# Intsights/PySubstringSearch

Measured on AMD Instinct MI355X. Metric: queries/sec (batched) + index-build GB/s on 512MB chunk, 1/2/4/8 GPU, higher is better.
Workload: dtype u64

## Files before the change

### pysubstringsearch_amd/csrc/msd_sort.hip

```cpp
#include "msd_sort.h"

#include <algorithm>
#include <type_traits>
#include <vector>

#include "prims.h"
#include "scan.h"
#include "text_keys.h"

namespace pss {

constexpr int MSD_D = 10;
constexpr u32 MSD_BINS = 1u << MSD_D;
constexpr int MSD_BLOCK = 512;
constexpr int MSD_WAVES = MSD_BLOCK / kWave;
constexpr int MSD_IPT = 16;
constexpr u32 MSD_TILE = MSD_BLOCK * MSD_IPT;
constexpr u32 MSD_WIN = 6144;
#ifndef PSS_LS_WINDOW
#define PSS_LS_WINDOW 8
#endif
constexpr u32 MSD_TILE_CAP = 8184 - PSS_LS_WINDOW;
constexpr u32 MSD_MAX_BUCKET = 4088;
constexpr int MSD_TAG_BITS = MSD_D + 1;
// ... 382 lines not shown
#pragma unroll
        for (int k = 0; k < MSD_IPT; ++k) {
            const u32 p = k * MSD_BLOCK + tid;
            if (p < valid) {
                u64 e = exch[p];
                u32 d;
                if (FROM_TEXT) {
                    d = (u32)(e >> 13) & (MSD_BINS - 1u);
                    e = ((e >> 23) << a.idx_bits) | (u64)(base + ((u32)e & (MSD_TILE - 1u)));
                } else {
                    d = (u32)(e >> shift2) & (MSD_BINS - 1u);
                    e = (e & low_mask2) | ((u64)(hist[d] >> 16) << shift2);
                }
                a.out[s_delta[d] + p] = e;
            }
        }
    }
}

constexpr u32 MSD_TILE2 = 16384;
constexpr int MSD_PIECES2 = MSD_TILE2 / MSD_TILE;

template <bool FROM_TEXT, int BLOCK, bool LSD = false>
__global__ __launch_bounds__(BLOCK) void msd_scatter2_kernel(MsdArgs a)
{
    constexpr int IPT = MSD_TILE2 / BLOCK;
    constexpr int BPT = MSD_BINS / BLOCK;
    __shared__ __attribute__((aligned(16))) u64 exch[MSD_TILE];
    __shared__ u32 hist[MSD_BINS], s_delta[MSD_BINS], s_off[MSD_BINS];
    __shared__ u16 s_start[MSD_BINS];
    __shared__ u32 scr[BLOCK / kWave + 1];
    const u32 tid = threadIdx.x, r = blockIdx.x;
    u32 e0, e1;
    u32 tag[BPT];
#pragma unroll
    for (int j = 0; j < BPT; ++j) tag[j] = 0;
    if (FROM_TEXT) {
        if (r >= a.num_ranges1) return;
        e0 = r * a.tiles_per_range1 * MSD_TILE;
        const u64 end = (u64)(r + 1) * a.tiles_per_range1 * MSD_TILE;
        e1 = end < a.n ? (u32)end : a.n;
    } else {
        if (r >= a.counters[0]) return;
        e0 = a.ranges2[r].start;
        e1 = a.ranges2[r].end;
#pragma unroll
        for (int j = 0; j < BPT; ++j)
            tag[j] = ((u32)a.dense[(size_t)a.ranges2[r].seg * MSD_BINS + BPT * tid + j] & (MSD_TAG_SPAN - 1u)) << 16;
    }
#pragma unroll
    for (int j = 0; j < BPT; ++j) {
        const u32 i = BPT * tid + j;
        hist[i] = tag[j];
        s_off[i] = FROM_TEXT ? a.T[(size_t)i * a.num_ranges1 + r] + a.J1[i] : a.T[(size_t)r * MSD_BINS + i];
    }
    __syncthreads();
    const int shift2 = a.idx_bits + a.key_bits - 2 * MSD_D;
    const u64 low_mask2 = (1ull << shift2) - 1ull;
    const int rest_bits = a.key_bits - MSD_D;
    const u64 rest_mask = (1ull << rest_bits) - 1ull;
    for (u32 base = e0; base < e1; base += MSD_TILE2) {
        const u32 valid = min(MSD_TILE2, e1 - base);
        u64 elem[IPT];
        u32 lp[IPT];
        if (FROM_TEXT) {
#pragma unroll
            for (int g = 0; g < IPT / 16; ++g) {
                const u32 i0 = base + tid * IPT + g * 16;
                u64 key[16] = {};
                if (i0 < a.n) text_keys16(a.codes, i0, a.code_bits, a.key_chars, a.plus_one, a.key_drop, a.n, key);
#pragma unroll
                for (int k = 0; k < 16; ++k) {
                    const u32 pos = tid * IPT + g * 16 + k;
                    u32 d;
                    u64 keep;
                    if (LSD) {
                        d = (u32)(key[k] >> (rest_bits - MSD_D)) & (MSD_BINS - 1u);
                        keep = ((key[k] >> rest_bits) << (rest_bits - MSD_D)) | (key[k] & (rest_mask >> MSD_D));
                    } else {
                        d = (u32)(key[k] >> rest_bits) & (MSD_BINS - 1u);
                        keep = key[k] & rest_mask;
                    }
                    elem[g * 16 + k] = (keep << 24) | ((u64)d << 14) | (u64)pos;
                    lp[g * 16 + k] = pos < valid ? ((atomicAdd(&hist[d], 1u) & 0xffffu) | (d << 22)) : 0xffffffffu;
                }
            }
        } else {
#pragma unroll
            for (int k = 0; k < IPT; ++k) {
                const u32 p = k * BLOCK + tid;
                elem[k] = p < valid ? a.in[base + p] : 0ull;
            }
#pragma unroll
            for (int k = 0; k < IPT; ++k) {
                const u32 p = k * BLOCK + tid;
                const u32 d = (u32)(elem[k] >> shift2) & (MSD_BINS - 1u);
                lp[k] = p < valid ? ((atomicAdd(&hist[d], 1u) & 0xffffu) | (d << 22)) : 0xffffffffu;
            }
        }
        __syncthreads();
        {
            u32 c[BPT], sum = 0;
#pragma unroll
            for (int j = 0; j < BPT; ++j) {
                c[j] = hist[BPT * tid + j] & 0xffffu;
                sum += c[j];
            }
            u32 ex = block_excl_sum<BLOCK / kWave>(sum, scr, nullptr);
#pragma unroll
            for (int j = 0; j < BPT; ++j) {
                const u32 i = BPT * tid + j;
                s_start[i] = (u16)ex;
                const u32 o = s_off[i];
                s_delta[i] = o - ex;
                s_off[i] = o + c[j];
                hist[i] = tag[j];
                ex += c[j];
            }
        }
        __syncthreads();
#pragma unroll
        for (int k = 0; k < IPT; ++k)
            if (lp[k] != 0xffffffffu) lp[k] = (lp[k] & 0xffffu) + (u32)s_start[lp[k] >> 22];
#pragma unroll
        for (int h = 0; h < MSD_PIECES2; ++h) {
            if (h * MSD_TILE >= valid) break;
            if (h) __syncthreads();
#pragma unroll
            for (int k = 0; k < IPT; ++k) {
                const u32 q = lp[k] - h * MSD_TILE;
                if (q < MSD_TILE) exch[q] = elem[k];
            }
            __syncthreads();
#pragma unroll
            for (int k = 0; k < (int)(MSD_TILE / BLOCK); ++k) {
                const u32 q = k * BLOCK + tid, p = h * MSD_TILE + q;
                if (p < valid) {
                    u64 e = exch[q];
                    u32 d;
                    if (FROM_TEXT) {
                        d = (u32)(e >> 14) & (MSD_BINS - 1u);
                        e = ((e >> 24) << a.idx_bits) | (u64)(base + ((u32)e & (MSD_TILE2 - 1u)));
                    } else {
                        d = (u32)(e >> shift2) & (MSD_BINS - 1u);
                        e = (e & low_mask2) | ((u64)(hist[d] >> 16) << shift2);
                    }
                    a.out[s_delta[d] + p] = e;
                }
            }
        }
    }
}

constexpr u32 LB_A = 1u << 30, LB_P = 2u << 30, LB_STATE = 3u << 30, LB_VALUE = LB_A - 1u;
constexpr int LB_WINDOW = 4;

struct LbAsk {
    u32 v[LB_WINDOW];
};
__device__ __forceinline__ void lb_ask(const u32 *status, u32 p, LbAsk &q)
{
#pragma unroll
    for (u32 w = 0; w < (u32)LB_WINDOW; ++w) {
        const u32 r = p > w ? p - 1 - w : 0u;
        q.v[w] = __hip_atomic_load(&status[(size_t)r * MSD_BINS + threadIdx.x], __ATOMIC_RELAXED, __HIP_MEMORY_SCOPE_AGENT);
    }
}
__device__ __forceinline__ void lb_begin(u32 *status, u32 t, u32 c, LbAsk &q)
{
    if (t == 0) return;
    __hip_atomic_store(&status[(size_t)t * MSD_BINS + threadIdx.x], LB_A | c, __ATOMIC_RELAXED, __HIP_MEMORY_SCOPE_AGENT);
    lb_ask(status, t, q);
}
__device__ __forceinline__ u32 lb_finish(u32 *status, u32 t, u32 c, u32 first, LbAsk &q)
{
    u32 off = first;
    if (t != 0) {
        u32 sum = 0, p = t;
        for (;;) {
            const u32 p0 = p;
            bool stop = false, done = false;
#pragma unroll
            for (u32 w = 0; w < (u32)LB_WINDOW; ++w) {
                if (!stop && w < p0) {
                    const u32 st = q.v[w] & LB_STATE;
                    if (st == 0) {
                        stop = true;
                    } else {
                        sum += q.v[w] & LB_VALUE;
                        --p;
                        if (st == LB_P) done = stop = true;
                    }
                }
            }
            if (done || p == 0) break;
            lb_ask(status, p, q);
        }
        off = sum;
    }
    __hip_atomic_store(&status[(size_t)t * MSD_BINS + threadIdx.x], LB_P | (off + c), __ATOMIC_RELAXED, __HIP_MEMORY_SCOPE_AGENT);
    return off;
}


__global__ __launch_bounds__(MSD_BINS) void msd_tiles2_kernel(const u32 *J1, MsdTile2 *tiles, u32 *counters)
{
    __shared__ u32 scr[MSD_BINS / kWave + 1];
    const u32 d = threadIdx.x;
    const u32 s = J1[d], e = J1[d + 1];
    const u32 nr = (e - s + MSD_TILE2 - 1) / MSD_TILE2;
    u32 total = 0, D = 0;
    const u32 first = block_excl_sum<MSD_BINS / kWave>(nr, scr, &total);
    const u32 dn = block_excl_sum<MSD_BINS / kWave>(nr ? 1u : 0u, scr, &D);
    if (d == 0) counters[0] = total + (MSD_BINS - D);
    if (nr == 0) {
        const u32 dd = D + (d - dn);
        tiles[total + (d - dn)] = MsdTile2{s, 0u, dd | 0x80000000u};
    }
    for (u32 k = 0; k < nr; ++k) {
        const u32 ts = s + k * MSD_TILE2;
        tiles[first + k] = MsdTile2{ts, min(MSD_TILE2, e - ts), dn | (k + 1 == nr ? 0x80000000u : 0u)};
    }
}

__global__ __launch_bounds__(1024) void msd_scatter_lb_kernel(MsdArgs a)
{
    constexpr int BLOCK = 1024;
    constexpr int IPT = MSD_TILE2 / BLOCK;
    __shared__ __attribute__((aligned(16))) u64 exch[MSD_TILE];
    __shared__ u32 hist[MSD_BINS], s_delta[MSD_BINS];
    __shared__ u16 s_start[MSD_BINS];
    __shared__ u32 scr[BLOCK / kWave + 1];
    __shared__ u32 s_ticket;
    const u32 tid = threadIdx.x;
    const u32 nt = a.counters[0];
    const int shift2 = a.idx_bits + a.key_bits - 2 * MSD_D;
    const u64 low_mask2 = (1ull << shift2) - 1ull;
    hist[tid] = 0;
    __syncthreads();
    for (;;) {
        if (tid == 0) s_ticket = atomicAdd(&a.counters[8], 1u);
        __syncthreads();
        const u32 t = s_ticket;
        if (t >= nt) break;
        const MsdTile2 td = a.tiles2[t];
        const u32 base = td.start, valid = td.count;
        u64 elem[IPT];
        u32 lp[IPT];
#pragma unroll
        for (int k = 0; k < IPT; ++k) {
            const u32 p = k * BLOCK + tid;
            elem[k] = p < valid ? a.in[base + p] : 0ull;
        }
#pragma unroll
        for (int k = 0; k < IPT; ++k) {
            const u32 p = k * BLOCK + tid;
            const u32 d = (u32)(elem[k] >> shift2) & (MSD_BINS - 1u);
            lp[k] = p < valid ? (atomicAdd(&hist[d], 1u) | (d << 22)) : 0xffffffffu;
        }
        __syncthreads();
        const u32 c = hist[tid];
        LbAsk ask;
        lb_begin(a.status, t, c, ask);
        const u32 ex = block_excl_sum<BLOCK / kWave>(c, scr, nullptr);
        s_start[tid] = (u16)ex;
        hist[tid] = 0;
        __syncthreads();
        const u64 tag = (u64)(td.d_last & (MSD_RAW_TAG_SPAN - 1u)) << shift2;
#pragma unroll
        for (int k = 0; k < IPT; ++k)
            if (lp[k] != 0xffffffffu) lp[k] = (lp[k] & 0xffffu) + (u32)s_start[lp[k] >> 22];
#pragma unroll
        for (int h = 0; h < MSD_PIECES2; ++h) {
            if (h && h * MSD_TILE >= valid) break;
            if (h) __syncthreads();
#pragma unroll
            for (int k = 0; k < IPT; ++k) {
                const u32 q = lp[k] - h * MSD_TILE;
                if (q < MSD_TILE) exch[q] = elem[k];
            }
            if (h == 0) {
                if (t == 0 && tid == 0) a.J[0] = 0;
                const u32 off = lb_finish(a.status, t, c, a.Jb[tid], ask);
                if (td.d_last >> 31) a.J[(size_t)tid * MSD_BINS + (td.d_last & (MSD_BINS - 1u)) + 1u] = off + c;
                s_delta[tid] = off - ex;
            }
            __syncthreads();
#pragma unroll
            for (int k = 0; k < (int)(MSD_TILE / BLOCK); ++k) {
                const u32 q = k * BLOCK + tid, p = h * MSD_TILE + q;
                if (p < valid) {
                    const u64 e = exch[q];
                    const u32 d = (u32)(e >> shift2) & (MSD_BINS - 1u);
                    a.out[s_delta[d] + p] = (e & low_mask2) | tag;
                }
            }
        }
    }
}


struct InNonEmpty {
    const u32 *J;
    __device__ u64 operator()(u64 j) const { return J[j + 1] > J[j] ? 1u : 0u; }
};

// ... 665 lines not shown

#include "ss_sort_impl.h"


static size_t msd_max_tiles(uint32_t n)
{
    return (size_t)n / (SS_WIN / 2) + ((size_t)MSD_BINS * MSD_BINS) / MSD_RAW_TAG_SPAN + 8;
}

static size_t msd_max_tiles2(uint32_t n) { return (size_t)n / MSD_TILE2 + MSD_BINS + 8; }

static bool msd_use_lsd(uint32_t n)
{
    const char *e = knob("PSS_MSD_LSD");
    return !(e && atoi(e) == 0) && n < (1u << 30);
}

size_t msd_workspace_bytes(uint32_t n)
{
    const size_t max_ranges2 = (size_t)n / MSD_G2_RANGE + MSD_BINS + 8;
    const size_t nbk = (size_t)MSD_BINS * MSD_BINS;
    return max_ranges2 * MSD_BINS * 4
           + (MSD_BINS + 8) * 4
           + (nbk + 8) * 4
           + max_ranges2 * sizeof(MsdRange) + (MSD_BINS + 8) * 4 + 64
           + (nbk + 8) * 8
           + (nbk + 8) * 4
           + (msd_max_tiles(n) + 32) * 8
           + (msd_max_tiles(n) + 32) * 16
           + (msd_max_tiles(n) + 32) * sizeof(MsdTile)
           + (SC_MAX_BLOCKS + 8) * 8 + 8192
           + (size_t)MSD_BINS * MSD_G1_RANGES * 4 + (MSD_BINS + 8) * 4
           + msd_max_tiles2(n) * (sizeof(MsdTile2) + (size_t)MSD_BINS * 4)
           + (nbk + 8) * 4 + 4096;
}

int msd_max_key_bits(uint32_t n)
{
    int ib = 1;
    while ((1ull << ib) < (u64)n) ++ib;
    const int after2 = 64 + MSD_D - (msd_use_lsd(n) ? MSD_RAW_TAG_BITS : MSD_TAG_BITS) - ib + MSD_D;
    return std::min(after2, 64 + MSD_D - ib);
}

int msd_suffix_sort(DeviceCtx *ctx, const TextKeys *text, uint32_t n, int key_bits, uint64_t *A[2], uint32_t *sa_out,
                    void *work, uint32_t *h_small, bool profile, MsdStats *stats, bool *accepted, MsdActive *active,
                    const MsdFront *front)
{
    *accepted = false;
    hipStream_t s = ctx->stream;
    int ib = 1;
    while ((1ull << ib) < (u64)n) ++ib;
    if (key_bits < 2 * MSD_D + 1 || key_bits > msd_max_key_bits(n) || n < 2) {
        set_error("msd_suffix_sort: key of %d bits does not fit (n = %u)", key_bits, n);
        return PSS_EINVAL;
    }
    const size_t max_ranges2 = (size_t)n / MSD_G2_RANGE + MSD_BINS + 8;
    const size_t nbk = (size_t)MSD_BINS * MSD_BINS;
    u8 *w = static_cast<u8 *>(work);
    size_t o = 0;
    auto carve = [&](size_t bytes) { u8 *p = w + o; o = round_up(o + bytes, 256); return p; };
    u32 *T = reinterpret_cast<u32 *>(carve(max_ranges2 * MSD_BINS * 4));
    u32 *J1 = reinterpret_cast<u32 *>(carve((MSD_BINS + 8) * 4));
    u32 *J = reinterpret_cast<u32 *>(carve((nbk + 8) * 4));
    MsdRange *ranges2 = reinterpret_cast<MsdRange *>(carve(max_ranges2 * sizeof(MsdRange)));
    u32 *seg_first = reinterpret_cast<u32 *>(carve((MSD_BINS + 8) * 4));
    u32 *counters = reinterpret_cast<u32 *>(carve(64));
    u64 *ranks = reinterpret_cast<u64 *>(carve((nbk + 8) * 8));
    u32 *cstart = reinterpret_cast<u32 *>(carve((nbk + 8) * 4));
    const size_t max_tiles = msd_max_tiles(n);
    MsdTile *tiles_all = reinterpret_cast<MsdTile *>(carve((max_tiles + 16) * sizeof(MsdTile)));
    u32 *tile_first = reinterpret_cast<u32 *>(carve((max_tiles + 16) * 8));
    u32 *blk_cnt = reinterpret_cast<u32 *>(carve((max_tiles + 8) * 4));
    u64 *dst_off = reinterpret_cast<u64 *>(carve((max_tiles + 8) * 8));
    u64 *partial = reinterpret_cast<u64 *>(carve((SC_MAX_BLOCKS + 8) * 8));
    u64 *d_total = partial + SC_MAX_BLOCKS;
    const bool lsd = msd_use_lsd(n);
    const size_t max_tiles2 = msd_max_tiles2(n);
    u32 *T2 = nullptr, *Jb = nullptr, *status = nullptr, *cj = nullptr;
    MsdTile2 *tiles2 = nullptr;
    if (lsd) {
        T2 = reinterpret_cast<u32 *>(carve((size_t)MSD_BINS * MSD_G1_RANGES * 4));
        Jb = reinterpret_cast<u32 *>(carve((MSD_BINS + 8) * 4));
        tiles2 = reinterpret_cast<MsdTile2 *>(carve(max_tiles2 * sizeof(MsdTile2)));
        status = reinterpret_cast<u32 *>(carve(max_tiles2 * MSD_BINS * 4));
        cj = reinterpret_cast<u32 *>(carve((nbk + 8) * 4));
    }

    MsdArgs a;
    memset(&a, 0, sizeof a);
    a.codes = text->codes;
    a.code_bits = text->code_bits;
    a.key_chars = text->key_chars;
    a.plus_one = text->plus_one;
    a.key_drop = text->drop;
    a.n = n;
    a.key_bits = key_bits;
    a.idx_bits = ib;
    const u32 num_tiles = (u32)(((u64)n + MSD_TILE - 1) / MSD_TILE);
    a.tiles_per_range1 = (num_tiles + MSD_G1_RANGES - 1) / MSD_G1_RANGES;
    a.num_ranges1 = (num_tiles + a.tiles_per_range1 - 1) / a.tiles_per_range1;
    a.T = T;
    a.J1 = J1;
    a.J = J;
    a.ranges2 = ranges2;
    a.seg_first = seg_first;
    a.counters = counters;
    a.lsd = lsd ? 1 : 0;
    a.T2 = T2;
    a.Jb = Jb;
    a.tiles2 = tiles2;
    a.status = status;

    hipEvent_t ev[8] = {};
    int nev = 0;
    struct EvGuard {
        hipEvent_t *e;
        int *n;
        ~EvGuard()
        {
            for (int i = 0; i < *n; ++i) (void)hipEventDestroy(e[i]);
        }
    } guard{ev, &nev};
    auto mark = [&]() -> int {
        if (profile && nev < 8) {
            PSS_HIP(hipEventCreate(&ev[nev]));
            PSS_HIP(hipEventRecord(ev[nev], s));
            ++nev;
        }
        return PSS_OK;
    };

    PSS_HIP(hipMemsetAsync(counters, 0, 64, s));
    a.out = A[0];
    if (front) {
        a.raw = front->raw;
        a.lut = front->lut;
        a.codes_out = const_cast<u8 *>(text->codes);
        a.bad = front->bad;
        hipLaunchKernelGGL(msd_hist_raw_kernel, dim3(a.num_ranges1), dim3(MSD_BLOCK), 0, s, a);
    } else {
        hipLaunchKernelGGL(msd_hist_kernel<true>, dim3(a.num_ranges1), dim3(MSD_BLOCK), 0, s, a);
    }
    static_assert(MSD_G1_RANGES <= 1024, "msd_offsets1_kernel takes four ranges per thread");
    hipLaunchKernelGGL(msd_offsets1_kernel, dim3(MSD_BINS), dim3(256), 0, s, T, a.num_ranges1, seg_first);
    hipLaunchKernelGGL(msd_offsets1b_kernel, dim3(1), dim3(MSD_BINS), 0, s, (const u32 *)seg_first, J1, n);
    if (lsd) {
        hipLaunchKernelGGL(msd_offsets1_kernel, dim3(MSD_BINS), dim3(256), 0, s, T2, a.num_ranges1, seg_first);
        hipLaunchKernelGGL(msd_offsets1b_kernel, dim3(1), dim3(MSD_BINS), 0, s, (const u32 *)seg_first, Jb, n);
        PSS_HIP(hipMemsetAsync(status, 0, max_tiles2 * MSD_BINS * 4, s));
    }
    PSS_TRY(mark());
    const bool wide = lsd || !(knob("PSS_MSD_SCATTER") && atoi(knob("PSS_MSD_SCATTER")) == 1);
    if (lsd) hipLaunchKernelGGL((msd_scatter2_kernel<true, 1024, true>), dim3(a.num_ranges1), dim3(1024), 0, s, a);
    else if (wide) hipLaunchKernelGGL((msd_scatter2_kernel<true, 1024>), dim3(a.num_ranges1), dim3(1024), 0, s, a);
    else hipLaunchKernelGGL(msd_scatter_kernel<true>, dim3(a.num_ranges1), dim3(MSD_BLOCK), 0, s, a);
    PSS_TRY(mark());
    a.in = A[0];
    a.out = A[1];
    if (lsd) {
        hipLaunchKernelGGL(msd_tiles2_kernel, dim3(1), dim3(MSD_BINS), 0, s, (const u32 *)J1, tiles2, counters);
        PSS_TRY(mark());
        const u32 grid2 = std::min<u32>((u32)max_tiles2, (u32)ctx->num_cus);
        hipLaunchKernelGGL(msd_scatter_lb_kernel, dim3(grid2), dim3(1024), 0, s, a);
        PSS_TRY(mark());
    } else {
        hipLaunchKernelGGL(msd_ranges_kernel, dim3(1), dim3(MSD_BINS), 0, s, J1, ranges2, seg_first, counters);
        a.dense = ranks;
        hipLaunchKernelGGL(msd_hist_kernel<false>, dim3((u32)max_ranges2), dim3(MSD_BLOCK), 0, s, a);
        hipLaunchKernelGGL(msd_offsets_kernel, dim3(MSD_BINS), dim3(MSD_BINS), 0, s, T, (const u32 *)seg_first, (const u32 *)J1, J,
                           0u, n, MSD_BINS);
    }
    PSS_TRY(device_excl_scan(ctx, InNonEmpty{J}, nbk, partial, d_total, ranks));
    hipLaunchKernelGGL(msd_compact_kernel, dim3(1024), dim3(256), 0, s, J, (u32)nbk, ranks, cstart, counters, cj);
    const int rem_bits = key_bits - 2 * MSD_D;
    MsdEmit em{};
    const int fused = active != nullptr;
    if (fused) em = MsdEmit{active->st_pos, active->st_idx, blk_cnt};
    const bool one_trip = lsd && !knob("PSS_MSD_SLOW_LOCAL");
    u64 *d_total2 = d_total + 1;
    u32 *const fail_list_dev = tile_first + max_tiles + 16;
    if (one_trip) {
        const TilePlan tpd{MSD_WIN, MSD_TILE_CAP, cj};
        PSS_TRY(device_excl_scan(ctx, InTileHeadDev{cstart, d_total, n, tpd}, nbk, partial, d_total2, ranks));
        hipLaunchKernelGGL(msd_tiles_dev_kernel, dim3(1024), dim3(256), 0, s, cstart, (const u64 *)d_total, n, ranks, (const u64 *)d_total2,
                           tile_first, tpd);
        hipLaunchKernelGGL(msd_tile_desc_kernel, dim3((u32)((max_tiles + 255) / 256)), dim3(256), 0, s, cstart, tile_first, 0u, 0u, n,
                           tiles_all, (const u32 *)cj, (const u64 *)d_total2, (const u64 *)d_total);
        PSS_TRY(mark());
        hipLaunchKernelGGL(msd_local_fast_kernel, dim3(2u * (u32)ctx->num_cus), dim3(MSD_BLOCK), 0, s, A[1], (const MsdTile *)tiles_all, 0u,
                           rem_bits, ib, sa_out, fail_list_dev, counters + 4, fused, em, (const u64 *)d_total2, (const u32 *)counters,
                           front ? (const u32 *)front->bad : (const u32 *)nullptr);
        PSS_TRY(mark());
        PSS_HIP(hipMemcpyAsync(h_small + 8, d_total2, 8, hipMemcpyDeviceToHost, s));
        PSS_HIP(hipMemcpyAsync(h_small + 10, counters + 4, 4, hipMemcpyDeviceToHost, s));
    }
    PSS_HIP(hipMemcpyAsync(h_small, d_total, 8, hipMemcpyDeviceToHost, s));
    PSS_HIP(hipMemcpyAsync(h_small + 2, counters, 16, hipMemcpyDeviceToHost, s));
    if (front) PSS_HIP(hipMemcpyAsync(h_small + 6, front->bad, 4, hipMemcpyDeviceToHost, s));
    PSS_HIP(hipStreamSynchronize(s));
    const u32 ne = h_small[0];
    const u32 maxb = h_small[3];
    if (stats) {
        stats->buckets = ne;
        stats->max_bucket = maxb;
        stats->bad_symbol = front ? h_small[6] : 0u;
    }
    if (front && h_small[6]) return PSS_OK;
    if (maxb > MSD_MAX_BUCKET) return PSS_OK;
    if (!lsd) {
        PSS_TRY(mark());
        if (wide) hipLaunchKernelGGL((msd_scatter2_kernel<false, 1024>), dim3((u32)max_ranges2), dim3(1024), 0, s, a);
        else hipLaunchKernelGGL(msd_scatter_kernel<false>, dim3((u32)max_ranges2), dim3(MSD_BLOCK), 0, s, a);
        PSS_TRY(mark());
    }
    const auto local_sort = msd_local_sort_kernel;
    const auto local_fast = msd_local_fast_kernel;
    u32 nt = 0;
    u32 *fail_list = fail_list_dev;
    if (one_trip) {
        nt = h_small[8];
        if ((size_t)nt > max_tiles) {
            set_error("msd_suffix_sort: %u tiles planned, tables hold %zu (internal error)", nt, max_tiles);
            return PSS_EDEVICE;
        }
        const u32 nfail = h_small[10];
        if (stats) stats->slow_tiles = nfail;
        if (nfail)
            hipLaunchKernelGGL(local_sort, dim3(nfail), dim3(MSD_BLOCK), 0, s, A[1], (const MsdTile *)tiles_all, rem_bits,
                               ib, sa_out, (const u32 *)fail_list, fused, em);
    } else {
    const TilePlan tp{MSD_WIN, MSD_TILE_CAP, cj};
    PSS_TRY(device_excl_scan(ctx, InTileHead{cstart, ne, n, tp}, ne, partial, d_total, ranks));
    hipLaunchKernelGGL(msd_tiles_kernel, dim3(1024), dim3(256), 0, s, cstart, ne, n, ranks, (const u64 *)d_total, tile_first, tp);
    PSS_HIP(hipMemcpyAsync(h_small, d_total, 8, hipMemcpyDeviceToHost, s));
    PSS_HIP(hipStreamSynchronize(s));
    nt = h_small[0];
    if ((size_t)nt > max_tiles) {
        set_error("msd_suffix_sort: %u tiles planned, tables hold %zu (internal error)", nt, max_tiles);
        return PSS_EDEVICE;
    }
    PSS_TRY(mark());
    fail_list = tile_first + nt + 8;
    hipLaunchKernelGGL(msd_tile_desc_kernel, dim3((nt + 255) / 256), dim3(256), 0, s, cstart, tile_first, nt, ne, n, tiles_all,
                       (const u32 *)cj, (const u64 *)nullptr, (const u64 *)nullptr);
    if (knob("PSS_MSD_SLOW_LOCAL")) {
        hipLaunchKernelGGL(local_sort, dim3(nt), dim3(MSD_BLOCK), 0, s, A[1], (const MsdTile *)tiles_all, rem_bits, ib,
                           sa_out, (const u32 *)nullptr, fused, em);
    } else {
        MsdTile *tiles = tiles_all;
        const u32 grid = std::min<u32>(nt, 2u * (u32)ctx->num_cus);
        hipLaunchKernelGGL(local_fast, dim3(grid), dim3(MSD_BLOCK), 0, s, A[1], (const MsdTile *)tiles, nt, rem_bits, ib,
                           sa_out, fail_list, counters + 4, fused, em, (const u64 *)nullptr, (const u32 *)nullptr, (const u32 *)nullptr);
        PSS_TRY(mark());
        PSS_HIP(hipMemcpyAsync(h_small, counters + 4, 4, hipMemcpyDeviceToHost, s));
        PSS_HIP(hipStreamSynchronize(s));
        const u32 nfail = h_small[0];
        if (stats) stats->slow_tiles = nfail;
        if (nfail)
            hipLaunchKernelGGL(local_sort, dim3(nfail), dim3(MSD_BLOCK), 0, s, A[1], (const MsdTile *)tiles_all, rem_bits,
                               ib, sa_out, (const u32 *)fail_list, fused, em);
    }
    if (knob("PSS_MSD_SLOW_LOCAL")) PSS_TRY(mark());
    }
    if (fused) {
        const bool finish = knob("PSS_MSD_NO_FINISH") == nullptr;
        if (finish) {
            const int ks = std::min(64 / text->code_bits, 16);
            const MsdFinish fin{text->codes, text->code_bits, ks, text->plus_one,
                                (u32)(text->drop ? text->key_chars - 1 : text->key_chars), n};
            hipLaunchKernelGGL(msd_finish_kernel, dim3((nt + 3) / 4), dim3(256), 0, s, (const MsdTile *)tiles_all, blk_cnt, nt,
                               active->st_pos, active->st_idx, sa_out, fin);
        }
        PSS_TRY(device_excl_scan(ctx, InBlkCnt{blk_cnt}, nt, partial, d_total, dst_off));
        hipLaunchKernelGGL(msd_gather_kernel, dim3((nt + 3) / 4), dim3(256), 0, s, (const MsdTile *)tiles_all, blk_cnt, dst_off, nt,
                           active->st_pos, active->st_idx, active->pos, active->idx, active->grp);
        PSS_HIP(hipMemcpyAsync(h_small, d_total, 8, hipMemcpyDeviceToHost, s));
        PSS_HIP(hipStreamSynchronize(s));
        active->count = h_small[0];
        if (stats) stats->finished = h_small[1];
    }
    PSS_HIP(hipGetLastError());
    if (stats) {
        stats->tiles = nt;
        stats->lookback = lsd ? 1u : 0u;
    }
    if (profile && nev >= 6) {
        PSS_HIP(hipStreamSynchronize(s));
        float ms = 0.f;
        PSS_HIP(hipEventElapsedTime(&ms, ev[0], ev[1]));
        if (stats) stats->ms_g1 = ms;
        PSS_HIP(hipEventElapsedTime(&ms, ev[2], ev[3]));
        if (stats) stats->ms_g2 = ms;
        PSS_HIP(hipEventElapsedTime(&ms, ev[4], ev[5]));
        if (stats) stats->ms_local = ms;
    }
    *accepted = true;
    return PSS_OK;
}


struct SsGeometry {
    u32 B1, B2, os, S;
    int ib, kc, key_bits;
    u64 plo, phi;
};
static bool ss_geometry(uint32_t n, uint32_t radix, SsGeometry *g)
{
// ... 270 lines not shown
```

### pysubstringsearch_amd/csrc/text_keys.h

```cpp
#pragma once
#include "prims.h"

namespace pss {

constexpr int TK_IPT = 16;

__device__ __forceinline__ void text_keys16(const u8 *codes, u32 i0, int b, int k, int plus_one, int drop, u32 n,
                                            u64 (&key)[TK_IPT])
{
    const uint4 *p = reinterpret_cast<const uint4 *>(codes + i0);
    const uint4 lo = p[0], hi = p[1];
    const u64 q0 = (u64)lo.x | ((u64)lo.y << 32), q1 = (u64)lo.z | ((u64)lo.w << 32);
    const u64 q2 = (u64)hi.x | ((u64)hi.y << 32), q3 = (u64)hi.z | ((u64)hi.w << 32);
    const u64 mask = (k * b >= 64) ? ~0ull : ((1ull << (k * b)) - 1ull);
    u64 win = 0;
#pragma unroll
    for (int j = 0; j < 16; ++j) {
        const u64 src = (j < 8) ? q0 : q1;
        u32 c = (u32)(src >> ((j & 7) * 8)) & 0xffu;
        if (plus_one) c = (i0 + j < n) ? c + 1u : 0u;
        if (j < k) win = (win << b) | c;
    }
    key[0] = win >> drop;
    u64 a0, a1, a2;
    if (k >= 16) { a0 = q2; a1 = q3; a2 = 0; }
    else if (k >= 8) { a0 = q1; a1 = q2; a2 = q3; }
    else { a0 = q0; a1 = q1; a2 = q2; }
    const int sh = (k & 7) * 8;
    u64 s0 = a0, s1 = a1;
    if (sh) {
        s0 = (a0 >> sh) | (a1 << (64 - sh));
        s1 = (a1 >> sh) | (a2 << (64 - sh));
    }
#pragma unroll
    for (int r = 1; r < TK_IPT; ++r) {
        const int j = r - 1;
        const u64 src = (j < 8) ? s0 : s1;
        u32 c = (u32)(src >> ((j & 7) * 8)) & 0xffu;
        if (plus_one) c = ((u64)i0 + j + k < n) ? c + 1u : 0u;
        win = ((win << b) | c) & mask;
        key[r] = win >> drop;
    }
}

__device__ __forceinline__ u64 text_key_at(const u8 *codes, u32 j, int b, int k, int plus_one, u32 n)
{
    const uint4 *q = reinterpret_cast<const uint4 *>(codes + (j & ~15u));
    const uint4 a = q[0], c = q[1];
    const u64 x0 = (u64)a.x | ((u64)a.y << 32), x1 = (u64)a.z | ((u64)a.w << 32);
    const u64 x2 = (u64)c.x | ((u64)c.y << 32), x3 = (u64)c.z | ((u64)c.w << 32);
    const bool up = (j & 8u) != 0;
    const u32 s8 = (j & 7u) * 8u;
    const u64 l0 = up ? x1 : x0, l1 = up ? x2 : x1, l2 = up ? x3 : x2;
    const u64 w0 = s8 ? (l0 >> s8) | (l1 << (64 - s8)) : l0;
    const u64 w1 = s8 ? (l1 >> s8) | (l2 << (64 - s8)) : l1;
    u64 key = 0;
#pragma unroll
    for (int c = 0; c < 16; ++c) {
        if (c < k) {
            u32 v = (u32)((c < 8 ? w0 : w1) >> ((c & 7) * 8)) & 0xffu;
            if (plus_one) v = ((u64)j + c < n) ? v + 1u : 0u;
            key = (key << b) | v;
        }
    }
    return key;
}

}
```

Before: 71.12.

## Add text-walk first-pass scatter kernel that regenerates suffix keys instead of holding them

Adds a new first-pass MSD scatter kernel that rebuilds each thread's 16 suffix keys on the fly with an incremental text walk. The keys are produced once for ranking and again for each exchange piece, so they are never kept in registers. Key-generation helpers are split into begin/step pieces to support this. The kernel is meant to cut register pressure and raise occupancy (launch bounds 1024,8), and PLUS_ONE becomes a template parameter. The cost is recomputing keys and reloading text per piece, and the step omits the window mask (~0ull is passed), which could change key bits if the window exceeds 64 bits.

```diff
diff --git a/pysubstringsearch_amd/csrc/msd_sort.hip b/pysubstringsearch_amd/csrc/msd_sort.hip
--- a/pysubstringsearch_amd/csrc/msd_sort.hip
+++ b/pysubstringsearch_amd/csrc/msd_sort.hip
@@ -558,6 +558,102 @@
     }
 }
 
+template <bool LSD, bool PLUS_ONE>
+__global__ __launch_bounds__(1024, 8) void msd_scatter_text_kernel(MsdArgs a)
+{
+    constexpr int BLOCK = 1024, IPT = MSD_TILE2 / BLOCK;
+    static_assert(IPT == TK_IPT && MSD_BINS == BLOCK, "one walk of 16 suffixes and one bin per thread");
+    __shared__ __attribute__((aligned(16))) u64 exch[MSD_TILE];
+    __shared__ u32 hist[MSD_BINS], s_delta[MSD_BINS], s_off[MSD_BINS];
+    __shared__ u16 s_start[MSD_BINS];
+    __shared__ u32 scr[BLOCK / kWave + 1];
+    const u32 tid0 = threadIdx.x, r = blockIdx.x;
+    if (r >= a.num_ranges1) return;
+    const u32 e0 = r * a.tiles_per_range1 * MSD_TILE;
+    const u64 end = (u64)(r + 1) * a.tiles_per_range1 * MSD_TILE;
+    const u32 e1 = end < a.n ? (u32)end : a.n;
+    hist[tid0] = 0;
+    s_off[tid0] = a.T[(size_t)tid0 * a.num_ranges1 + r] + a.J1[tid0];
+    __syncthreads();
+    const int rest_bits = a.key_bits - MSD_D;
+    const u64 rest_mask = (1ull << rest_bits) - 1ull;
+    const int sh_top = a.key_drop + rest_bits;
+    const int sh_d = LSD ? sh_top - MSD_D : sh_top;
+    const u64 low_mask = LSD ? rest_mask >> MSD_D : rest_mask;
+    for (u32 base = e0; base < e1; base += MSD_TILE2) {
+        const u32 valid = min(MSD_TILE2, e1 - base);
+        u32 tid = tid0;
+        int kc = a.key_chars;
+        asm volatile("" : "+v"(tid), "+s"(kc));
+        const u32 i0 = base + tid * IPT;
+        TextWalk w = {0, 0, 0};
+        if (i0 < a.n) w = text_walk_begin(a.codes, i0, a.code_bits, kc, PLUS_ONE, a.n);
+        auto walk = [&](auto f) __attribute__((always_inline)) {
+            u32 t = tid;
+            asm volatile("" : "+v"(w.win), "+v"(w.s0), "+v"(w.s1), "+v"(t));
+            u64 win = w.win;
+#pragma unroll
+            for (int k = 0; k < IPT; ++k) {
+                if (k) win = text_walk_step(win, w, k, base + t * IPT, a.code_bits, kc, PLUS_ONE, a.n, ~0ull);
+                f(k, t * IPT + k, win);
+            }
+        };
+        u32 lp[IPT];
+        auto rank = [&](auto full) __attribute__((always_inline)) {
+            walk([&](int k, u32 pos, u64 win) __attribute__((always_inline)) {
+                const u32 d = (u32)(win >> sh_d) & (MSD_BINS - 1u);
+                lp[k] = decltype(full)::value || pos < valid ? ((atomicAdd(&hist[d], 1u) & 0xffffu) | (d << 22)) : 0xffffffffu;
+            });
+        };
+        if (valid == MSD_TILE2) rank(std::true_type{});
+        else rank(std::false_type{});
+        __syncthreads();
+        {
+            const u32 c = hist[tid];
+            const u32 incl = wave_incl_sum_dpp(c);
+            const u32 wave_no = (u32)__builtin_amdgcn_readfirstlane((int)(tid >> 6));
+            if ((tid & (kWave - 1u)) == kWave - 1u) scr[wave_no] = incl;
+            __syncthreads();
+            u32 ex = incl - c;
+#pragma unroll
+            for (u32 wv = 0; wv + 1 < (u32)(BLOCK / kWave); ++wv) ex += wv < wave_no ? scr[wv] : 0u;
+            s_start[tid] = (u16)ex;
+            const u32 o = s_off[tid];
+            s_delta[tid] = o - ex;
+            s_off[tid] = o + c;
+            hist[tid] = 0;
+        }
+        __syncthreads();
+#pragma unroll
+        for (int k = 0; k < IPT; ++k) {
+            const u32 start = s_start[lp[k] >> 22];
+            lp[k] = lp[k] == 0xffffffffu ? lp[k] : (lp[k] & 0xffffu) + start;
+        }
+#pragma unroll
+        for (int h = 0; h < MSD_PIECES2; ++h) {
+            if (h * MSD_TILE >= valid) break;
+            if (h) __syncthreads();
+            walk([&](int k, u32 pos, u64 win) __attribute__((always_inline)) {
+                const u32 q = lp[k] - h * MSD_TILE;
+                const u32 d = (u32)(win >> sh_d) & (MSD_BINS - 1u);
+                u64 keep = (win >> a.key_drop) & low_mask;
+                if (LSD) keep |= ((win >> sh_top) & (u64)(MSD_BINS - 1u)) << (rest_bits - MSD_D);
+                if (q < MSD_TILE) exch[q] = (keep << 24) | ((u64)d << 14) | (u64)pos;
+            });
+            __syncthreads();
+#pragma unroll
+            for (int k = 0; k < (int)(MSD_TILE / BLOCK); ++k) {
+                const u32 q = k * BLOCK + tid, p = h * MSD_TILE + q;
+                if (p < valid) {
+                    const u64 e = exch[q];
+                    const u32 d = (u32)(e >> 14) & (MSD_BINS - 1u);
+                    a.out[s_delta[d] + p] = ((e >> 24) << a.idx_bits) | (u64)(base + ((u32)e & (MSD_TILE2 - 1u)));
+                }
+            }
+        }
+    }
+}
+
 constexpr u32 LB_A = 1u << 30, LB_P = 2u << 30, LB_STATE = 3u << 30, LB_VALUE = LB_A - 1u;
 constexpr int LB_WINDOW = 4;
 
@@ -1529,8 +1625,11 @@
     }
     PSS_TRY(mark());
     const bool wide = lsd || !(knob("PSS_MSD_SCATTER") && atoi(knob("PSS_MSD_SCATTER")) == 1);
-    if (lsd) hipLaunchKernelGGL((msd_scatter2_kernel<true, 1024, true>), dim3(a.num_ranges1), dim3(1024), 0, s, a);
-    else if (wide) hipLaunchKernelGGL((msd_scatter2_kernel<true, 1024>), dim3(a.num_ranges1), dim3(1024), 0, s, a);
+    if (wide) {
+        auto *const first_pass = lsd ? (a.plus_one ? msd_scatter_text_kernel<true, true> : msd_scatter_text_kernel<true, false>)
+                                     : (a.plus_one ? msd_scatter_text_kernel<false, true> : msd_scatter_text_kernel<false, false>);
+        hipLaunchKernelGGL(first_pass, dim3(a.num_ranges1), dim3(1024), 0, s, a);
+    }
     else hipLaunchKernelGGL(msd_scatter_kernel<true>, dim3(a.num_ranges1), dim3(MSD_BLOCK), 0, s, a);
     PSS_TRY(mark());
     a.in = A[0];
diff --git a/pysubstringsearch_amd/csrc/text_keys.h b/pysubstringsearch_amd/csrc/text_keys.h
--- a/pysubstringsearch_amd/csrc/text_keys.h
+++ b/pysubstringsearch_amd/csrc/text_keys.h
@@ -5,40 +5,62 @@
 
 constexpr int TK_IPT = 16;
 
-__device__ __forceinline__ void text_keys16(const u8 *codes, u32 i0, int b, int k, int plus_one, int drop, u32 n,
-                                            u64 (&key)[TK_IPT])
+struct TextWalk {
+    u64 win;
+    u64 s0, s1;
+};
+
+__device__ __forceinline__ TextWalk text_walk_begin(const u8 *codes, u32 i0, int b, int k, int plus_one, u32 n)
 {
     const uint4 *p = reinterpret_cast<const uint4 *>(codes + i0);
     const uint4 lo = p[0], hi = p[1];
     const u64 q0 = (u64)lo.x | ((u64)lo.y << 32), q1 = (u64)lo.z | ((u64)lo.w << 32);
     const u64 q2 = (u64)hi.x | ((u64)hi.y << 32), q3 = (u64)hi.z | ((u64)hi.w << 32);
-    const u64 mask = (k * b >= 64) ? ~0ull : ((1ull << (k * b)) - 1ull);
-    u64 win = 0;
+    TextWalk w;
+    w.win = 0;
 #pragma unroll
     for (int j = 0; j < 16; ++j) {
         const u64 src = (j < 8) ? q0 : q1;
         u32 c = (u32)(src >> ((j & 7) * 8)) & 0xffu;
         if (plus_one) c = (i0 + j < n) ? c + 1u : 0u;
-        if (j < k) win = (win << b) | c;
+        if (j < k) w.win = (w.win << b) | c;
     }
-    key[0] = win >> drop;
     u64 a0, a1, a2;
     if (k >= 16) { a0 = q2; a1 = q3; a2 = 0; }
     else if (k >= 8) { a0 = q1; a1 = q2; a2 = q3; }
     else { a0 = q0; a1 = q1; a2 = q2; }
     const int sh = (k & 7) * 8;
-    u64 s0 = a0, s1 = a1;
+    w.s0 = a0;
+    w.s1 = a1;
     if (sh) {
-        s0 = (a0 >> sh) | (a1 << (64 - sh));
-        s1 = (a1 >> sh) | (a2 << (64 - sh));
+        w.s0 = (a0 >> sh) | (a1 << (64 - sh));
+        w.s1 = (a1 >> sh) | (a2 << (64 - sh));
     }
+    return w;
+}
+
+__device__ __forceinline__ u64 text_walk_step(u64 win, const TextWalk &w, int r, u32 i0, int b, int k, int plus_one, u32 n,
+                                              u64 mask)
+{
+    const int j = r - 1;
+    const u64 src = (j < 8) ? w.s0 : w.s1;
+    u32 c = (u32)(src >> ((j & 7) * 8)) & 0xffu;
+    if (plus_one) c = ((u64)i0 + j + k < n) ? c + 1u : 0u;
+    return ((win << b) | c) & mask;
+}
+
+__device__ __forceinline__ u64 text_walk_mask(int b, int k) { return (k * b >= 64) ? ~0ull : ((1ull << (k * b)) - 1ull); }
+
+__device__ __forceinline__ void text_keys16(const u8 *codes, u32 i0, int b, int k, int plus_one, int drop, u32 n,
+                                            u64 (&key)[TK_IPT])
+{
+    const TextWalk w = text_walk_begin(codes, i0, b, k, plus_one, n);
+    const u64 mask = text_walk_mask(b, k);
+    u64 win = w.win;
+    key[0] = win >> drop;
 #pragma unroll
     for (int r = 1; r < TK_IPT; ++r) {
-        const int j = r - 1;
-        const u64 src = (j < 8) ? s0 : s1;
-        u32 c = (u32)(src >> ((j & 7) * 8)) & 0xffu;
-        if (plus_one) c = ((u64)i0 + j + k < n) ? c + 1u : 0u;
-        win = ((win << b) | c) & mask;
+        win = text_walk_step(win, w, r, i0, b, k, plus_one, n, mask);
         key[r] = win >> drop;
     }
 }
```

Measured after the change: 71.79 (median of 6 runs). No clear change (+0.9%).
